# QData/LaMP

Hardware: AMD Instinct MI355X
Metric: forward samples/sec, reuters d512 2+2L 4h (higher is better)
Workload: dtype f32

## Files before the change

### lamp_amd/csrc/chain.hip

```cpp
#include "lamp_asm.h"

namespace lamp {

namespace {
constexpr int ROWS = 16;
constexpr int BK = 32;

}

struct ChainGemm {
    const float* W[3];
    const float* Wp[3];
    const float* Wq[3];
    const float* bias[3];
    float* C[3];
    int nseg, N, K;
    int64_t ldw, ldc;
    int relu;
    int src;
    int dst;
    int add_dst;
};
struct ChainLN {
    const float* g;
// ... 770 lines not shown
    auto buf_f = [&](int which) { return smem + (which ? x_floats : 0); };
    auto buf_w = [&](int which) { return which ? p.hw : d; };

    int pc = 0;
    auto first = [&]() { return (wave - pc) & (WAVES - 1); };
    auto load_rows = [&](const float* src, int64_t ld, int width, int which) {
        const __amdgpu_buffer_rsrc_t rs = rsrc_u(src + row0 * ld, (uint64_t(rows_m - 1) * uint64_t(ld) + uint64_t(width)) * 4u);
        const int ppr = width / 256, n = R * ppr;
        float* dst = buf_f(which);
        const int rl = buf_w(which);
        for (int k = first(); k < n; k += WAVES) {
            const int r = k / ppr, part = k - r * ppr;
            const unsigned voff = unsigned(r) * unsigned(ld) * 4u + unsigned(part * 64 + (lane ^ (r & 15))) * 16u;
            lds_dma16(rs, dst + r * rl + part * 256, r < rows_m ? voff : OOB, 0);
        }
        pc += n;
    };
    auto load_vec = [&](const float* src, int n_floats, int at) {
        const __amdgpu_buffer_rsrc_t rs = rsrc_u(src, uint64_t(n_floats) * 4u);
        const int n = n_floats / 256;
        for (int k = first(); k < n; k += WAVES) lds_dma16(rs, smem + at + k * 256, unsigned(k * 64 + lane) * 16u, 0);
        pc += n;
    };
    auto load_mod_rows = [&](const float* table, int mod, int at, int ld) {
        const __amdgpu_buffer_rsrc_t rs = rsrc_u(table, uint64_t(mod) * uint64_t(d) * 4u);
        const int ppr = d / 256, n = R * ppr;
        for (int k = first(); k < n; k += WAVES) {
            const int r = k / ppr, part = k - r * ppr;
            const unsigned src_row = unsigned(row0 + r) % unsigned(mod);
            lds_dma16(rs, smem + at + r * ld + part * 256, r < rows_m ? (src_row * unsigned(d) + unsigned(part * 64 + lane) * 4u) * 4u : OOB, 0);
        }
        pc += n;
    };
    if (p.in_x) load_rows(p.in_x, d, d, 0);
    load_rows(p.in_h, p.ld_h, p.k_h, 1);
    load_vec(p.ln1.g, d, c_g1);
    load_vec(p.ln1.b, d, c_be1);
    if (p.ln1.res) load_mod_rows(p.ln1.res, p.ln1.r_mod, c_res, res_ld);
    const ChainLN& lnl = p.has_ffn ? p.ln2 : p.ln1;
    if (p.has_ffn) {
        load_vec(p.ln2.g, d, c_g2);
        load_vec(p.ln2.b, d, c_be2);
        load_vec(p.w2.bias[0], d, c_b2);
        load_vec(p.w1.bias[0], dff, c_b1);
    }
    if (lnl.w_out && !p.wout_late) load_mod_rows(lnl.w_out, lnl.n_labels, c_wout, d);
    wait_vmcnt<0>();
    wg_barrier();

#ifdef LAMP_TUNING
    unsigned long long gt[3][4] = {};
    int gt_i = 0;
#endif
    auto gemm = [&](const ChainGemm& g, int bias_at) {
        CHAIN_STAMP(0);
        const int nc = g.K / 16, npass = g.N / 512, total = npass * nc;
        const unsigned w_bytes = unsigned(g.N) * unsigned(g.K) * 4u;
        u32x4 rsW = raw_rsrc(g.Wq[0], w_bytes);
        const unsigned f_voff = unsigned(lane) * 16u;
        const unsigned pass_jump = 7u * unsigned(nc) * 4096u + 4096u;
        unsigned s_off = unsigned(wave) * unsigned(nc) * 4096u;
        int pt = 0, p_kt = 0, p_wrap = 0;
        auto adv_a = [&]() { ++pt; ++p_kt; p_wrap = p_kt == nc ? 1 : 0; };
        auto adv_b = [&]() { s_off += p_wrap ? pass_jump : 4096u; p_kt = p_wrap ? 0 : p_kt; };
        auto adv_c = [&]() {
#if defined(CHAIN_ABL) && (CHAIN_ABL & 1)
            rsW[2] = 0u;
#else
            rsW[2] = pt < total ? w_bytes : 0u;
#endif
        };
        auto wload = [&](f32x4& dst, auto Q) { dst = buffer_read16_untracked_off<decltype(Q)::value * 1024>(rsW, f_voff, s_off); };
        f32x4 F[DEPTH][4];
        float fa[2][G];
        unsigned a_cur[G];
        const unsigned src_b = buf_b(g.src), row_bytes = unsigned(buf_w(g.src)) * 4u;
        const int bq = lane >> 4, be = (lane >> 2) & 3;
        auto a_lane = [&](int gg) { return src_b + unsigned(4 * gg + l3) * row_bytes + unsigned((bq ^ l3) << 4) + unsigned(be) * 4u; };
#pragma unroll
        for (int gg = 0; gg < G; ++gg) a_cur[gg] = a_lane(gg);
        auto aread = [&](auto SET, auto GG, auto J) {
            constexpr int set = decltype(SET)::value, gg = decltype(GG)::value, j = decltype(J)::value;
            fa[set][gg] = lds_read4_off<64 * (j ^ (gg & 3))>(a_cur[gg]);
        };
        static_for<0, DEPTH - 1>([&](auto J) {
            constexpr int j = decltype(J)::value;
            sgpr_guard(rsW, s_off);
            static_for<0, 4>([&](auto Q) { wload(F[j][decltype(Q)::value], Q); });
            adv_a(); adv_b(); adv_c();
        });
        static_for<0, G>([&](auto GG) { aread(std::integral_constant<int, 0>{}, GG, std::integral_constant<int, 0>{}); });
        wait_vmcnt<(DEPTH - 2) * 4>();
        wait_lgkmcnt<0>();
        CHAIN_STAMP(1);
        for (int pass = 0; pass < npass; ++pass) {
            const int col = pass * 512 + wave * 64 + lane;
            f32x4 acc[G];
#pragma unroll
            for (int gg = 0; gg < G; ++gg) acc[gg] = f32x4{0.f, 0.f, 0.f, 0.f};
            for (int kt0 = 0; kt0 < nc; kt0 += DEPTH) {
                const unsigned q_next = unsigned(kt0 + DEPTH == nc ? 0 : (kt0 + DEPTH) >> 2) * 256u;
                static_for<0, DEPTH>([&](auto J) {
                    constexpr int j = decltype(J)::value, set = j & 1, setn = (j + 1) & 1;
                    constexpr int jl = (j + DEPTH - 1) % DEPTH, jn = (j + 1) % DEPTH;
                    static_for<0, NMF>([&](auto I) {
                        constexpr int i = decltype(I)::value, jj = i / (4 * G), q = (i / G) % 4, gg = i % G;
#if !(defined(CHAIN_ABL) && (CHAIN_ABL & 2))
                        acc[gg] = __builtin_amdgcn_mfma_f32_4x4x1f32(fa[set][gg], F[j][q][jj], acc[gg], 4, 4 * q + jj, 0);
#endif
                        __builtin_amdgcn_sched_barrier(0);
                        if constexpr (i < 8 && i % 2 == 0) {
#if !(defined(CHAIN_ABL) && (CHAIN_ABL & 16))
                            wload(F[jl][i / 2], std::integral_constant<int, i / 2>{});
#endif
                        } else if constexpr (i < 2 * G && i % 2 == 1 && i != NMF - 1) {
#if !(defined(CHAIN_ABL) && (CHAIN_ABL & 8))
                            aread(std::integral_constant<int, setn>{}, std::integral_constant<int, i / 2>{}, std::integral_constant<int, jn>{});
#endif
                        } else if constexpr (i == 8) {
                            adv_a();
                        } else if constexpr (i == 10) {
                            adv_b();
                        } else if constexpr (i == 12) {
                            adv_c();
                        } else if constexpr (i >= 14 && i % 2 == 0 && (i - 14) / 2 < G && j == DEPTH - 2) {
                            a_cur[(i - 14) / 2] = a_lane((i - 14) / 2) + q_next;
                        } else if constexpr (i == NMF - 1) {
                            asm volatile("s_waitcnt vmcnt(%0) lgkmcnt(0)" ::"n"((DEPTH - 2) * 4) : "memory");
                        }
                        __builtin_amdgcn_sched_barrier(0);
                    });
                });
            }
            if (pass + 1 == npass) wait_vmcnt<0>();
            static_for<0, DEPTH - 1>([&](auto J) { static_for<0, 4>([&](auto Q) { keep_alive(F[decltype(J)::value][decltype(Q)::value]); }); });
            static_for<0, G>([&](auto GG) { keep_alive(fa[0][decltype(GG)::value]); });
            CHAIN_STAMP(2);
            const unsigned drow = unsigned(buf_w(g.dst)) * 4u;
            float rv[G][4];
            unsigned at[G][4];
#pragma unroll
            for (int gg = 0; gg < G; ++gg)
#pragma unroll
                for (int i = 0; i < 4; ++i) {
                    const int r = 4 * gg + i;
                    at[gg][i] = buf_b(g.dst) + unsigned(r) * drow + unsigned(((col >> 2) ^ (r & 15)) << 4) + unsigned(col & 3) * 4u;
                    rv[gg][i] = lds_read4(at[gg][i]);
                }
            float bias_v = lds_read4(bias_at >= 0 ? lds0 + unsigned(bias_at + col) * 4u : at[0][0]);
            wait_lgkmcnt<0>();
            settle(bias_v);
#pragma unroll
            for (int gg = 0; gg < G; ++gg)
#pragma unroll
                for (int i = 0; i < 4; ++i) settle(rv[gg][i]);
            const float bias = bias_at >= 0 ? bias_v : 0.f;
#pragma unroll
            for (int gg = 0; gg < G; ++gg)
#pragma unroll
                for (int i = 0; i < 4; ++i) {
                    float v = acc[gg][i] + bias;
                    if (g.relu) v = fmaxf(v, 0.f);
                    if (g.add_dst) v = v + rv[gg][i];
                    lds_write4(at[gg][i], v);
                }
        }
        wait_vmcnt<0>();
        wg_barrier();
        CHAIN_STAMP(3);
#ifdef LAMP_TUNING
        ++gt_i;
#endif
    };

    auto layernorm = [&](const ChainLN& n, int g_at, int be_at) {
        const int nv = d / 4;
        int cq[NV];
#pragma unroll
        for (int i = 0; i < NV; ++i) cq[i] = lane + i * 64 < nv ? lane + i * 64 : nv - 1;
#pragma unroll
        for (int q = 0; q < RPW; ++q) {
            const int r = wave + q * WAVES;
            if (r < R) {
                const bool live = r < rows_m;
                const int64_t row = row0 + (live ? r : 0);
                const unsigned row_b = lds0 + unsigned(r) * unsigned(d) * 4u;
                f32x4 raw[NV], gg[NV], bb[NV], rr[NV], ww[NV];
#pragma unroll
                for (int i = 0; i < NV; ++i) {
                    const unsigned self = row_b + unsigned((cq[i] ^ (r & 15)) << 4);
                    raw[i] = lds_read16(self);
                    gg[i] = lds_read16(lds0 + unsigned(g_at) * 4u + unsigned(cq[i]) * 16u);
                    bb[i] = lds_read16(lds0 + unsigned(be_at) * 4u + unsigned(cq[i]) * 16u);
                    rr[i] = lds_read16(n.res ? lds0 + unsigned(c_res + r * res_ld) * 4u + unsigned(cq[i]) * 16u : self);
                    ww[i] = lds_read16(n.w_out ? lds0 + unsigned(c_wout + r * d) * 4u + unsigned(cq[i]) * 16u : self);
                }
                wait_lgkmcnt<0>();
#pragma unroll
                for (int i = 0; i < NV; ++i) {
                    settle(raw[i]); settle(gg[i]); settle(bb[i]); settle(rr[i]); settle(ww[i]);
// ... 5 lines not shown
                    v[i] = in ? make_float4(raw[i].x, raw[i].y, raw[i].z, raw[i].w) : make_float4(0.f, 0.f, 0.f, 0.f);
                    if (n.res && in) {
                        v[i].x += rr[i].x; v[i].y += rr[i].y; v[i].z += rr[i].z; v[i].w += rr[i].w;
                    }
                }
                float mean, rstd;
                ln_row_stats<NV>(v, lane, nv, d, n.eps, mean, rstd);
                float4* yr = (n.y && live) ? reinterpret_cast<float4*>(n.y + row * d) : nullptr;
                float dot = 0.f;
#pragma unroll
                for (int i = 0; i < NV; ++i) {
                    if (lane + i * 64 < nv) {
                        const float4 o = ln_row_apply(v[i], mean, rstd, make_float4(gg[i].x, gg[i].y, gg[i].z, gg[i].w),
                                                      make_float4(bb[i].x, bb[i].y, bb[i].z, bb[i].w));
                        lds_write16(row_b + unsigned((cq[i] ^ (r & 15)) << 4), f32x4{o.x, o.y, o.z, o.w});
                        if (yr) yr[cq[i]] = o;
                        if (n.w_out) dot += dot4_nocontract(o, make_float4(ww[i].x, ww[i].y, ww[i].z, ww[i].w));
                    }
                }
                if (n.w_out) {
                    dot = wave64_sum(dot);
                    if (lane == 0 && live) n.logits[row] = dot;
                }
            }
        }
        wg_barrier();
    };

#ifdef LAMP_TUNING
    unsigned long long t[6] = {};
    const unsigned long long c_begin = __builtin_readcyclecounter();
    if (p.trace) t[0] = wall_clock64();
#endif
    gemm(p.fc, -1);
#ifdef LAMP_TUNING
    if (p.trace) t[1] = wall_clock64();
#endif
    layernorm(p.ln1, c_g1, c_be1);
#ifdef LAMP_TUNING
    if (p.trace) t[2] = wall_clock64();
#endif
    if (p.has_ffn) {
        gemm(p.w1, c_b1);
#ifdef LAMP_TUNING
        if (p.trace) t[3] = wall_clock64();
#endif
        gemm(p.w2, c_b2);
#ifdef LAMP_TUNING
        if (p.trace) t[4] = wall_clock64();
#endif
        if (p.wout_late) {
            load_mod_rows(p.ln2.w_out, p.ln2.n_labels, c_wout, d);
            wait_vmcnt<0>();
            wg_barrier();
        }
        layernorm(p.ln2, c_g2, c_be2);
    }
#ifdef LAMP_TUNING
    if (p.trace && tid == 0) {
        unsigned long long* o = p.trace + size_t(blockIdx.x) * 24;
        t[5] = wall_clock64();
        for (int i = 0; i < 6; ++i) o[i] = t[i];
        o[6] = __builtin_readcyclecounter() - c_begin;
        o[7] = __builtin_amdgcn_s_getreg((31 << 11) | 20);
        for (int gi = 0; gi < 3; ++gi)
            for (int k = 0; k < 4; ++k) o[8 + gi * 4 + k] = gt[gi][k] - c_begin;
    }
#endif
}

#ifdef LAMP_TUNING
static unsigned long long* g_chain_trace = nullptr;
extern "C" __attribute__((visibility("default"))) void lamp_debug_set_chain_trace(unsigned long long* buf) { g_chain_trace = buf; }
static int g_chain_mode = -1;
extern "C" __attribute__((visibility("default"))) void lamp_debug_force_chain(int mode) { g_chain_mode = mode; }
static int g_chain_geom = -1;
extern "C" __attribute__((visibility("default"))) void lamp_debug_chain_geometry(int idx) { g_chain_geom = idx; }
#endif

#define LAMP_CHAIN_GEOMS(X) X(0, 16, 32, 2, 1) X(1, 8, 32, 4, 2) X(2, 8, 32, 2, 2) X(3, 8, 32, 4, 1) X(4, 8, 64, 2, 1) \
// ... 248 lines not shown
```

### lamp_amd/csrc/attention_small.hip

```cpp
#include "lamp_kernels.h"

namespace lamp {

#ifndef LAMP_LDS_PAD16
#define LAMP_LDS_PAD16 8
#endif
constexpr int ATTN16_PAD = LAMP_LDS_PAD16;

namespace {
__device__ __forceinline__ void swap16(float& a, float& b) {
    asm volatile("s_nop 3\n\tv_permlane16_swap_b32 %0, %1\n\ts_nop 3" : "+v"(a), "+v"(b));
}
__device__ __forceinline__ void swap32(float& a, float& b) {
    asm volatile("s_nop 3\n\tv_permlane32_swap_b32 %0, %1\n\ts_nop 3" : "+v"(a), "+v"(b));
}
__device__ __forceinline__ float group_max(float v) {
    float a = v, b = v;
    swap16(a, b);
    a = fmaxf(a, b);
    b = a;
    swap32(a, b);
    return fmaxf(a, b);
}
__device__ __forceinline__ float group_sum(float v) {
    float a = v, b = v;
    swap16(a, b);
    a = a + b;
    b = a;
    swap32(a, b);
    return a + b;
}
}

// ... 277 lines not shown

    if (qi < p.lq) {
        float* Orow = p.O + int64_t(b) * p.lay.o_b + int64_t(h) * p.lay.o_h + int64_t(qi) * p.lay.o_r;
        const bool vec = ((p.lay.o_b | p.lay.o_h | p.lay.o_r) & 3) == 0 && (reinterpret_cast<uintptr_t>(p.O) & 15u) == 0;
#pragma unroll
        for (int r = 0; r < 4; ++r) {
#pragma unroll
            for (int e0 = 0; e0 < DV8; e0 += DVW) {
                const int col = DVW * (4 * g + r) + 64 * (e0 / DVW);
                if (col >= p.dv) continue;
                if (DVW == 4 && vec) {
                    *reinterpret_cast<float4*>(Orow + col) =
                        make_float4(o[e0][r] * inv_l, o[e0 + (DVW > 1 ? 1 : 0)][r] * inv_l,
                                    o[e0 + (DVW > 2 ? 2 : 0)][r] * inv_l, o[e0 + (DVW > 3 ? 3 : 0)][r] * inv_l);
                } else {
#pragma unroll
                    for (int e = 0; e < DVW; ++e) Orow[col + e] = o[e0 + e][r] * inv_l;
                }
            }
        }
    }
#ifdef LAMP_TUNING
    if (p.trace && tid == 0) {
        unsigned long long* t = p.trace + size_t(blockIdx.x) * 8;
        t[0] = t_entry; t[1] = t_loop; t[2] = t_merge; t[3] = wall_clock64();
        t[4] = __builtin_amdgcn_s_getreg((31 << 11) | 4);
        t[5] = __builtin_amdgcn_s_getreg((31 << 11) | 20);
        t[6] = unsigned(item);
        t[7] = unsigned(ks) | (unsigned(qb) << 8);
    }
#endif
}

template <int DP, int QB, int KSPLIT, int PM, int MK>
static int launch_small_mk(const AttnParams& p, hipStream_t s) {
    constexpr int NW = QB * KSPLIT;
    constexpr size_t lds_q = size_t(QB + NW) * 16 * (DP + ATTN16_PAD) * sizeof(float);
    constexpr size_t lds_c = KSPLIT > 1 ? size_t(NW) * (DP / 16 * 4 + 4) * 64 * sizeof(float) : 0;
    constexpr size_t lds = lds_q > lds_c ? lds_q : lds_c;
    auto kern = attn16_kernel<DP, QB, KSPLIT, PM, MK>;
    if constexpr (lds > 65536) {
        static AttrOnce once;
        if (int e = once.set(reinterpret_cast<const void*>(kern), lds)) return e;
    }
    const int64_t nwg = int64_t((p.lq + 16 * QB - 1) / (16 * QB)) * p.H * p.B;
    if (nwg > 0x7fffffffLL) return LAMP_E_DIMS;
    hipLaunchKernelGGL(kern, dim3(unsigned(nwg)), dim3(NW * 64), lds, s, p);
    return int(hipGetLastError());
}

template <int DP, int QB, int KSPLIT, int PM>
static int launch_small_ks(const AttnParams& p, hipStream_t s) {
    switch (p.mask_kind) {
        case LAMP_MASK_U8: return launch_small_mk<DP, QB, KSPLIT, PM, LAMP_MASK_U8>(p, s);
        case LAMP_MASK_KEY_TOKENS_I64: return launch_small_mk<DP, QB, KSPLIT, PM, LAMP_MASK_KEY_TOKENS_I64>(p, s);
        case LAMP_MASK_BITS_U32: return launch_small_mk<DP, QB, KSPLIT, PM, LAMP_MASK_BITS_U32>(p, s);
        default: return launch_small_mk<DP, QB, KSPLIT, PM, LAMP_MASK_NONE>(p, s);
    }
}

template <int DP, int QB, int KSPLIT>
static int launch_small_pm(const AttnParams& p, hipStream_t s) {
    return p.lse ? launch_small_ks<DP, QB, KSPLIT, 2>(p, s) : launch_small_ks<DP, QB, KSPLIT, 0>(p, s);
}

template <int DP>
static int launch_small_dp(const AttnParams& p, int qb, int ksplit, hipStream_t s) {
    switch (qb * 8 + ksplit) {
        case 1 * 8 + 1: return launch_small_pm<DP, 4, 1>(p, s);
        case 2 * 8 + 1: return launch_small_pm<DP, 4, 1>(p, s);
        case 3 * 8 + 1: return launch_small_pm<DP, 4, 1>(p, s);
        case 4 * 8 + 1: return launch_small_pm<DP, 4, 1>(p, s);
        case 1 * 8 + 2: return launch_small_pm<DP, 2, 2>(p, s);
        case 2 * 8 + 2: return launch_small_pm<DP, 2, 2>(p, s);
        case 3 * 8 + 2: return launch_small_pm<DP, 3, 2>(p, s);
        case 4 * 8 + 2: return launch_small_pm<DP, 4, 2>(p, s);
        case 1 * 8 + 4: return launch_small_pm<DP, 1, 4>(p, s);
        case 2 * 8 + 4: return launch_small_pm<DP, 2, 4>(p, s);
        case 3 * 8 + 4: return launch_small_pm<DP, 3, 4>(p, s);
        default: return launch_small_pm<DP, 2, 4>(p, s);
    }
}

bool attn_small_applies(const AttnParams& p, bool any_lq) {
    const bool few_keys = p.lk <= 64 && !p.kv_len;
    return (p.lq <= 256 || few_keys || any_lq) && p.V && p.O && (!p.P || p.lse) && p.dk <= 128 && p.dv <= 128;
}

#ifdef LAMP_TUNING
static unsigned long long* g_attn_trace = nullptr;
extern "C" __attribute__((visibility("default"))) void lamp_debug_set_attn_trace(unsigned long long* buf) { g_attn_trace = buf; }
#endif

int launch_attn_small(const AttnParams& p_in, int force, hipStream_t s) {
    AttnParams p = p_in;
    p.trace = nullptr;
#ifdef LAMP_TUNING
    p.trace = g_attn_trace;
#endif
    const int nt = (p.lk + 15) / 16;
    const int nqb = (p.lq + 15) / 16;
    int ksplit = force & 7;
    if (ksplit != 1 && ksplit != 2 && ksplit != 4) ksplit = nt >= 12 ? 4 : (nt >= 4 ? 2 : 1);
    int qb = (force >> 4) & 7;
    if (qb < 1 || qb > 4) qb = 4 / ksplit;
    (void)nqb;
    const int dmax = p.dk > p.dv ? p.dk : p.dv;
    if (dmax <= 32) return launch_small_dp<32>(p, qb, ksplit, s);
    if (dmax <= 64) return launch_small_dp<64>(p, qb, ksplit, s);
    return launch_small_dp<128>(p, qb, ksplit, s);
}

}
```

### lamp_amd/csrc/attention_tile.hip

```cpp
#include "lamp_asm.h"

namespace lamp {
namespace {

constexpr int TILE_FLOATS = 32 * 128;
constexpr int BUF_FLOATS = 2 * TILE_FLOATS;
constexpr int MAX_LIST_TILES = 2048;
constexpr size_t LDS_BYTES = size_t(2) * BUF_FLOATS * 4;
constexpr size_t LDS_BYTES_LIST = LDS_BYTES + (MAX_LIST_TILES / 32) * 4 + MAX_LIST_TILES * 4;

__device__ __forceinline__ void dma16(u32x4 rs, unsigned lds_addr, unsigned voff, unsigned soff) {
    asm volatile("s_mov_b32 m0, %0\n\ts_nop 0\n\tbuffer_load_dwordx4 %1, %2, %3 offen lds" ::"s"(lds_addr), "v"(voff), "s"(rs), "s"(soff)
                 : "memory");
}

template <int MK>
__global__ __launch_bounds__(256, 2) void attn_tile_kernel(AttnParams p) {
    static_assert(MK == LAMP_MASK_NONE || MK == LAMP_MASK_BITS_U32, "the plan's masks");
    constexpr int DKC = 16, DVB = 4;
    extern __shared__ __attribute__((aligned(16))) float smem[];
#ifdef TILE_TRACE
    const unsigned long long t_entry = wall_clock64();
#endif
    const int tid = threadIdx.x, lane = tid & 63, wave = __builtin_amdgcn_readfirstlane(tid >> 6);
    const int l31 = lane & 31, hi = lane >> 5;
    const int nqb = (p.lq + 127) / 128;
    const int item = xcd_remap(blockIdx.x, gridDim.x);
    const int qblk = item % nqb, bh = item / nqb;
    const int h = bh % p.H, b = bh / p.H;
    const int q0 = (qblk * 4 + wave) * 32;
    const int qi = q0 + l31;
    const bool wave_active = q0 < p.lq;
    const int qc = qi < p.lq ? qi : p.lq - 1;

    const int q_r = int(p.lay.q_r), k_r = int(p.lay.k_r), v_r = int(p.lay.v_r);
    const int lk_b = __builtin_amdgcn_readfirstlane(p.kv_len ? p.kv_len[b] : p.lk);
    const int row0 = __builtin_amdgcn_readfirstlane(p.kv_len ? p.kv_off[b] : 0);
    const int64_t k_row0 = p.kv_len ? int64_t(row0) * k_r : int64_t(b) * p.lay.k_b;
    const int64_t v_row0 = p.kv_len ? int64_t(row0) * v_r : int64_t(b) * p.lay.v_b;
    const __amdgpu_buffer_rsrc_t rsQ = make_rsrc(p.Q + int64_t(b) * p.lay.q_b + int64_t(h) * p.lay.q_h,
                                                 (uint64_t(p.lq - 1) * q_r + p.dk) * 4u);
    const u32x4 rsK = raw_rsrc(p.K + k_row0 + int64_t(h) * p.lay.k_h, lk_b > 0 ? unsigned((uint64_t(lk_b - 1) * k_r + p.dk) * 4u) : 0u);
    const u32x4 rsV = raw_rsrc(p.V + v_row0 + int64_t(h) * p.lay.v_h, lk_b > 0 ? unsigned((uint64_t(lk_b - 1) * v_r + p.dv) * 4u) : 0u);
    const u32x4 rsM = MK == LAMP_MASK_BITS_U32
                          ? raw_rsrc(reinterpret_cast<const float*>(static_cast<const unsigned*>(p.mask) + int64_t(b) * p.m_sb),
                                     unsigned((uint64_t(p.lq - 1) * uint64_t(p.m_sq) + (p.lk + 31) / 32) * 4u))
                          : raw_rsrc(p.K, 0u);
// ... 330 lines not shown
```

### lamp_amd/csrc/lamp_asm.h

```cpp
#pragma once
#include <type_traits>

#include "lamp_kernels.h"

namespace lamp {
namespace {
typedef __attribute__((address_space(3))) void* lds_ptr;
__device__ __forceinline__ void lds_dma16(__amdgpu_buffer_rsrc_t rs, float* dst, unsigned voff, unsigned soff) {
    __builtin_amdgcn_raw_ptr_buffer_load_lds(rs, (lds_ptr)dst, 16, voff, soff, 0, 0);
}
__device__ __forceinline__ f32x4 lds_read16(unsigned addr) {
    f32x4 v;
    asm volatile("ds_read_b128 %0, %1" : "=v"(v) : "v"(addr));
    return v;
}
__device__ __forceinline__ f32x4 global_read16_untracked(const float* ptr) {
    f32x4 v;
    asm volatile("global_load_dwordx4 %0, %1, off" : "=v"(v) : "v"(ptr) : "memory");
    return v;
}
typedef unsigned u32x4 __attribute__((ext_vector_type(4)));
__device__ __forceinline__ u32x4 raw_rsrc(const float* base, unsigned bytes) {
    const uint64_t b = reinterpret_cast<uint64_t>(base);
    return u32x4{unsigned(__builtin_amdgcn_readfirstlane(unsigned(b))), unsigned(__builtin_amdgcn_readfirstlane(unsigned(b >> 32) & 0xffffu)),
                 unsigned(__builtin_amdgcn_readfirstlane(bytes)), 0x00020000u};
}
__device__ __forceinline__ f32x4 buffer_read16_untracked(u32x4 rs, unsigned voff, unsigned soff) {
    f32x4 v;
    asm volatile("buffer_load_dwordx4 %0, %1, %2, %3 offen" : "=v"(v) : "v"(voff), "s"(rs), "s"(soff) : "memory");
    return v;
}
__device__ __forceinline__ void lds_write16(unsigned addr, f32x4 v) { asm volatile("ds_write_b128 %0, %1" ::"v"(addr), "v"(v) : "memory"); }
template <int I, int N, typename F>
__device__ __forceinline__ void static_for(F&& f) {
    if constexpr (I < N) {
        f(std::integral_constant<int, I>{});
        static_for<I + 1, N>(f);
    }
}
template <int N>
__device__ __forceinline__ void wait_vmcnt() { asm volatile("s_waitcnt vmcnt(%0)" ::"n"(N) : "memory"); }
template <int N>
__device__ __forceinline__ void wait_lgkmcnt() {
    asm volatile("s_waitcnt lgkmcnt(%0)" ::"n"(N) : "memory");
    __builtin_amdgcn_sched_barrier(0);
}
__device__ __forceinline__ void wg_barrier() {
    asm volatile("s_waitcnt lgkmcnt(0)" ::: "memory");
    __builtin_amdgcn_s_barrier();
    asm volatile("" ::: "memory");
    __builtin_amdgcn_sched_barrier(0);
}
__device__ __forceinline__ const float* uniform_ptr(const float* q) {
    const uint64_t b = reinterpret_cast<uint64_t>(q);
    const unsigned lo = __builtin_amdgcn_readfirstlane(unsigned(b)), hi = __builtin_amdgcn_readfirstlane(unsigned(b >> 32));
    return reinterpret_cast<const float*>((uint64_t(hi) << 32) | lo);
}
__device__ __forceinline__ __amdgpu_buffer_rsrc_t rsrc_u(const float* base, uint64_t bytes) {
// ... 48 lines not shown
```

### lamp_amd/isa_guard.py

```python
import os
import re
import subprocess
import sys
import tempfile

HIPCC = os.environ.get('HIPCC') or '/opt/rocm/bin/hipcc'

LOAD = re.compile(r'^\s*(buffer_load_dword\w*|global_load_dword\w*|ds_read\w*)\s+(v\[\d+:\d+\]|v\d+)\s*,\s*(.*)$')
REG = re.compile(r'v\[(\d+):(\d+)\]|v(\d+)')


def regs_of(text):
    out = set()
    for m in REG.finditer(text):
        if m.group(3) is not None:
            out.add(int(m.group(3)))
        else:
            out.update(range(int(m.group(1)), int(m.group(2)) + 1))
    return out


def device_asm(path, extra=()):
    if path.endswith('.s'):
        return open(path).read()
# ... 120 lines not shown
            continue
        ops = t.split(None, 1)
        if len(ops) < 2 or ops[0].startswith('s_'):
            continue
        operands = ops[1].split(';')[0]
        parts = [p.strip() for p in operands.split(',')]
        is_store = ops[0].startswith(('ds_write', 'buffer_store', 'global_store', 'scratch_store', 'buffer_load'))
        srcs = pk_sources(parts) if ops[0].startswith('v_pk_') else regs_of(','.join(parts if is_store else parts[1:]))
        dsts = set() if is_store else regs_of(parts[0])
        for regs, lno, ltxt in all_pending():
            if regs & srcs:
                findings.append((kernel, lno, ltxt, no, t))
            elif regs & dsts:
                findings.append((kernel, lno, ltxt, no, t + '   ; WRITES a register in flight'))
    return kernels, n_loads, findings


def m0_findings(asm):
    lines = [l.strip() for l in asm.split('\n')]
    uses = [i for i, l in enumerate(lines) if re.search(r'\bm0\b', l) and not l.startswith(';')]
    bad = []
    for i in uses:
        ok = (lines[i].startswith('s_mov_b32 m0, s') and i + 2 < len(lines) and lines[i + 1].startswith('s_nop') and
              lines[i + 2].startswith('buffer_load_dwordx4') and lines[i + 2].endswith('lds'))
        if not ok:
            bad.append((i + 1, lines[i]))
    n_dma = sum(l.endswith(' lds') and l.startswith('buffer_load') for l in lines)
    if n_dma != len(uses):
        bad.append((0, '%d LDS-DMA loads for %d m0 writes' % (n_dma, len(uses))))
    return len(uses), bad


GUARDED = {'chain.hip': (('chain',), 12, 500, False), 'slab.hip': (('slab',), 1, 500, False),
           'attention_tile.hip': (('attn_tile',), 2, 3, True)}


def guard_unit(path, flags=()):
    unit = os.path.basename(path)
    wanted, min_kernels, min_loads, owns_m0 = GUARDED[unit]
    asm = device_asm(path, flags)
    kernels, loads, findings = check(asm, wanted)
    out = ['%s: line %d `%s` <- line %d `%s`' % (k[:80], lno, ltxt, no, t) for k, lno, ltxt, no, t in findings]
    if kernels < min_kernels or loads <= min_loads:
        out.append('%s: only %d kernels / %d inline-assembly loads seen: the checker no longer recognises the unit' % (unit, kernels, loads))
    if owns_m0:
        n, bad = m0_findings(asm)
        out += ['%s: m0 at line %d: %s' % (unit, no, t) for no, t in bad]
        if n <= 20:
            out.append('%s: only %d m0 writes seen' % (unit, n))
    return out


def main():
    path = sys.argv[1] if len(sys.argv) > 1 else 'lamp_amd/csrc/chain.hip'
    wanted = tuple(sys.argv[2:]) or ('chain', 'slab')
    kernels, n_loads, findings = check(device_asm(path), wanted)
    print('%d kernels, %d inline-assembly loads checked, %d findings' % (kernels, n_loads, len(findings)))
    for k, lno, ltxt, no, t in findings[:40]:
        print('  %s\n    line %d: %s\n    line %d: %s' % (k[:90], lno, ltxt, no, t))
    sys.exit(1 if findings else 0)


if __name__ == '__main__':
    main()
```

Before: 46950.

## Prefetch next GEMM's weight tiles across chain stages and hoist first prefetch

Moves the weight register pipeline F out of the gemm lambda so its prologue prefetch for the first GEMM is issued before the activation/LN-parameter loads. At the tail of each GEMM the buffer descriptor switches to the next GEMM's weights, so the first DEPTH-1 tiles of the following GEMM stream in during the epilogue and layernorm rather than after a full drain. This hides cold-start weight latency between chained stages. The cost is more complex descriptor logic and in-flight loads held across barriers and layernorm, which raises register pressure and adds a correctness risk around the vmcnt waits.

```diff
diff --git a/lamp_amd/csrc/chain.hip b/lamp_amd/csrc/chain.hip
--- a/lamp_amd/csrc/chain.hip
+++ b/lamp_amd/csrc/chain.hip
@@ -826,6 +826,21 @@
         }
         pc += n;
     };
+    f32x4 F[DEPTH][4];
+    auto w_rsrc = [&](const ChainGemm& g, bool live) { return raw_rsrc(g.Wq[0], live ? unsigned(g.N) * unsigned(g.K) * 4u : 0u); };
+    auto w_first = [&](const ChainGemm& g) { return unsigned(wave) * unsigned(g.K / 16) * 4096u; };
+    {
+        const u32x4 rs = w_rsrc(p.fc, true);
+        const unsigned s0 = w_first(p.fc);
+        static_for<0, DEPTH - 1>([&](auto J) {
+            constexpr int j = decltype(J)::value;
+            const unsigned so = s0 + unsigned(j) * 4096u;
+            sgpr_guard(rs, so);
+            static_for<0, 4>([&](auto Q) {
+                F[j][decltype(Q)::value] = buffer_read16_untracked_off<decltype(Q)::value * 1024>(rs, unsigned(lane) * 16u, so);
+            });
+        });
+    }
     if (p.in_x) load_rows(p.in_x, d, d, 0);
     load_rows(p.in_h, p.ld_h, p.k_h, 1);
     load_vec(p.ln1.g, d, c_g1);
@@ -846,26 +861,30 @@
     unsigned long long gt[3][4] = {};
     int gt_i = 0;
 #endif
-    auto gemm = [&](const ChainGemm& g, int bias_at) {
+    auto gemm = [&](const ChainGemm& g, int bias_at, const ChainGemm& nx, bool has_next) {
         CHAIN_STAMP(0);
         const int nc = g.K / 16, npass = g.N / 512, total = npass * nc;
         const unsigned w_bytes = unsigned(g.N) * unsigned(g.K) * 4u;
-        u32x4 rsW = raw_rsrc(g.Wq[0], w_bytes);
+        u32x4 rsW = w_rsrc(g, true);
+        const u32x4 rsN = w_rsrc(nx, has_next);
+        const unsigned n_first = w_first(nx);
         const unsigned f_voff = unsigned(lane) * 16u;
         const unsigned pass_jump = 7u * unsigned(nc) * 4096u + 4096u;
-        unsigned s_off = unsigned(wave) * unsigned(nc) * 4096u;
-        int pt = 0, p_kt = 0, p_wrap = 0;
+        unsigned s_off = w_first(g) + unsigned(DEPTH - 1) * 4096u;
+        int pt = DEPTH - 1, p_kt = DEPTH - 1, p_wrap = 0;
         auto adv_a = [&]() { ++pt; ++p_kt; p_wrap = p_kt == nc ? 1 : 0; };
-        auto adv_b = [&]() { s_off += p_wrap ? pass_jump : 4096u; p_kt = p_wrap ? 0 : p_kt; };
+        auto adv_b = [&]() { s_off = pt == total ? n_first : s_off + (p_wrap ? pass_jump : 4096u); p_kt = p_wrap ? 0 : p_kt; };
         auto adv_c = [&]() {
+            const bool past = pt >= total;
+            rsW[0] = past ? rsN[0] : rsW[0];
+            rsW[1] = past ? rsN[1] : rsW[1];
 #if defined(CHAIN_ABL) && (CHAIN_ABL & 1)
             rsW[2] = 0u;
 #else
-            rsW[2] = pt < total ? w_bytes : 0u;
+            rsW[2] = past ? rsN[2] : w_bytes;
 #endif
         };
         auto wload = [&](f32x4& dst, auto Q) { dst = buffer_read16_untracked_off<decltype(Q)::value * 1024>(rsW, f_voff, s_off); };
-        f32x4 F[DEPTH][4];
         float fa[2][G];
         unsigned a_cur[G];
         const unsigned src_b = buf_b(g.src), row_bytes = unsigned(buf_w(g.src)) * 4u;
@@ -877,12 +896,6 @@
             constexpr int set = decltype(SET)::value, gg = decltype(GG)::value, j = decltype(J)::value;
             fa[set][gg] = lds_read4_off<64 * (j ^ (gg & 3))>(a_cur[gg]);
         };
-        static_for<0, DEPTH - 1>([&](auto J) {
-            constexpr int j = decltype(J)::value;
-            sgpr_guard(rsW, s_off);
-            static_for<0, 4>([&](auto Q) { wload(F[j][decltype(Q)::value], Q); });
-            adv_a(); adv_b(); adv_c();
-        });
         static_for<0, G>([&](auto GG) { aread(std::integral_constant<int, 0>{}, GG, std::integral_constant<int, 0>{}); });
         wait_vmcnt<(DEPTH - 2) * 4>();
         wait_lgkmcnt<0>();
@@ -926,7 +939,7 @@
                     });
                 });
             }
-            if (pass + 1 == npass) wait_vmcnt<0>();
+            if (pass + 1 == npass && !has_next) wait_vmcnt<0>();
             static_for<0, DEPTH - 1>([&](auto J) { static_for<0, 4>([&](auto Q) { keep_alive(F[decltype(J)::value][decltype(Q)::value]); }); });
             static_for<0, G>([&](auto GG) { keep_alive(fa[0][decltype(GG)::value]); });
             CHAIN_STAMP(2);
@@ -959,7 +972,6 @@
                     lds_write4(at[gg][i], v);
                 }
         }
-        wait_vmcnt<0>();
         wg_barrier();
         CHAIN_STAMP(3);
 #ifdef LAMP_TUNING
@@ -1031,7 +1043,7 @@
     const unsigned long long c_begin = __builtin_readcyclecounter();
     if (p.trace) t[0] = wall_clock64();
 #endif
-    gemm(p.fc, -1);
+    gemm(p.fc, -1, p.w1, p.has_ffn != 0);
 #ifdef LAMP_TUNING
     if (p.trace) t[1] = wall_clock64();
 #endif
@@ -1040,11 +1052,11 @@
     if (p.trace) t[2] = wall_clock64();
 #endif
     if (p.has_ffn) {
-        gemm(p.w1, c_b1);
+        gemm(p.w1, c_b1, p.w2, true);
 #ifdef LAMP_TUNING
         if (p.trace) t[3] = wall_clock64();
 #endif
-        gemm(p.w2, c_b2);
+        gemm(p.w2, c_b2, p.w2, false);
 #ifdef LAMP_TUNING
         if (p.trace) t[4] = wall_clock64();
 #endif
```

After: 47150, median of 6. Within noise of the previous version (+0.4%).

## Add LDS-staged small attention kernel sharing K/V tiles across query blocks via DMA

Applied to the files above, without the earlier changes.

Adds a new small-attention kernel in which each key-split wave group loads K/V tiles into LDS through buffer-load-to-LDS DMA and a double/triple-buffered ring. Three query blocks then read the same tile, so K/V global traffic is no longer repeated per query block. This becomes the default path when there is no LSE output and the key split is greater than one. In exchange it adds more LDS use per workgroup, barriers on every step in the non-burst case, and a fixed QB=3 choice; the ISA guard is extended to cover the new m0 usage.

```diff
diff --git a/lamp_amd/csrc/attention_small.hip b/lamp_amd/csrc/attention_small.hip
--- a/lamp_amd/csrc/attention_small.hip
+++ b/lamp_amd/csrc/attention_small.hip
@@ -1,4 +1,4 @@
-#include "lamp_kernels.h"
+#include "lamp_asm.h"
 
 namespace lamp {
 
@@ -342,6 +342,308 @@
 #endif
 }
 
+template <int DP, int QB, int KSPLIT, int NBUF, int MK>
+__global__ __launch_bounds__(QB* KSPLIT * 64) void attn16_lds_kernel(AttnParams p) {
+    static_assert(KSPLIT > 1 && NBUF >= 2, "shared tiles need a key split; the ring needs two buffers");
+    constexpr int DKC = DP / 16, DV8 = DP / 16;
+    constexpr int QS = DP + ATTN16_PAD;
+    constexpr int C4 = DP / 4, RPI = 64 / C4;
+    constexpr int SWM = (C4 < 16 ? C4 : 16) - 1;
+    constexpr int TILE = 16 * DP;
+    constexpr int NREQ = TILE * 4 / 1024;
+    constexpr int QFL = QB * 16 * QS;
+    extern __shared__ __attribute__((aligned(16))) float smem[];
+
+    const int tid = threadIdx.x;
+    const int lane = tid & 63, wave = __builtin_amdgcn_readfirstlane(tid >> 6);
+    const int l15 = lane & 15, g = lane >> 4;
+    const int rot = (p.kv_len) ? int(blockIdx.x % KSPLIT) : 0;
+    const int qb = wave / KSPLIT, ks = __builtin_amdgcn_readfirstlane((wave % KSPLIT + KSPLIT - rot) % KSPLIT);
+    const int slot = qb * KSPLIT + ks;
+#ifdef LAMP_TUNING
+    const unsigned long long t_entry = p.trace ? wall_clock64() : 0ull;
+    unsigned long long t_loop = 0, t_merge = 0;
+#endif
+    const int nqg = (p.lq + 16 * QB - 1) / (16 * QB);
+    const int item = xcd_remap(blockIdx.x, gridDim.x);
+    const int qgrp = item % nqg;
+    const int bh = item / nqg;
+    const int h = bh % p.H, b = bh / p.H;
+    const int q0 = (qgrp * QB + qb) * 16;
+    const int qi = q0 + l15;
+    const bool wave_active = q0 < p.lq;
+    const int qc = qi < p.lq ? qi : p.lq - 1;
+
+    const int q_r = int(p.lay.q_r), k_r = int(p.lay.k_r), v_r = int(p.lay.v_r);
+    const int lk_b = __builtin_amdgcn_readfirstlane(p.kv_len ? p.kv_len[b] : p.lk);
+    const int row0 = __builtin_amdgcn_readfirstlane(p.kv_len ? p.kv_off[b] : 0);
+    const int64_t k_row0 = p.kv_len ? int64_t(row0) * k_r : int64_t(b) * p.lay.k_b;
+    const int64_t v_row0 = p.kv_len ? int64_t(row0) * v_r : int64_t(b) * p.lay.v_b;
+    const __amdgpu_buffer_rsrc_t rsQ = make_rsrc(p.Q + int64_t(b) * p.lay.q_b + int64_t(h) * p.lay.q_h,
+                                                 (uint64_t(p.lq - 1) * q_r + p.dk) * 4u);
+    const u32x4 rsK = raw_rsrc(p.K + k_row0 + int64_t(h) * p.lay.k_h, lk_b > 0 ? unsigned((uint64_t(lk_b - 1) * k_r + p.dk) * 4u) : 0u);
+    const u32x4 rsV = raw_rsrc(p.V + v_row0 + int64_t(h) * p.lay.v_h, lk_b > 0 ? unsigned((uint64_t(lk_b - 1) * v_r + p.dv) * 4u) : 0u);
+    const __amdgpu_buffer_rsrc_t rsM =
+        MK == LAMP_MASK_BITS_U32
+            ? make_rsrc(static_cast<const unsigned*>(p.mask) + int64_t(b) * p.m_sb,
+                        (uint64_t(p.lq - 1) * uint64_t(p.m_sq) + (p.lk + 31) / 32) * 4u)
+        : MK == LAMP_MASK_U8
+            ? make_rsrc(static_cast<const unsigned char*>(p.mask) + int64_t(b) * p.m_sb,
+                        uint64_t(p.lq - 1) * uint64_t(p.m_sq) + p.lk)
+        : MK == LAMP_MASK_KEY_TOKENS_I64
+            ? make_rsrc(static_cast<const long long*>(p.mask) + int64_t(b) * p.m_sb, uint64_t(p.lk) * 8u)
+            : make_rsrc(p.K, 0);
+
+    const int nt_b = (lk_b + 15) / 16;
+    const int nt = nt_b;
+    const int ks_eff = p.kv_len ? (nt_b >= 12 ? (KSPLIT < 4 ? KSPLIT : 4) : (nt_b >= 4 ? 2 : 1)) : KSPLIT;
+    const int nsteps = nt > 0 ? (nt + ks_eff - 1) / ks_eff : 0;
+    const bool burst = nsteps <= NBUF;
+
+    unsigned kvo[NREQ];
+#pragma unroll
+    for (int i = 0; i < NREQ; ++i) {
+        const int r = i * RPI + lane / C4, q = (lane % C4) ^ (r & SWM);
+        kvo[i] = 4 * q < p.dk ? unsigned((lane / C4) * k_r + 4 * q) * 4u : OOB;
+    }
+    const unsigned vvo = 4 * (lane % C4) < p.dv ? unsigned((lane / C4) * v_r + 4 * (lane % C4)) * 4u : OOB;
+    auto buf_of = [&](int u) { return QFL + (ks * NBUF + u) * 2 * TILE; };
+    auto dma_tile = [&](int j, int u) {
+        const int kt = ks + j * ks_eff;
+        if (ks >= ks_eff || kt >= nt) return;
+        const unsigned base = unsigned(buf_of(u)) * 4u;
+#pragma unroll
+        for (int n = 0; n < 2 * NREQ; ++n) {
+            if (n % QB != qb) continue;
+            if (n < NREQ) dma16(rsK, base + 1024u * n, kvo[n], unsigned((kt * 16 + n * RPI) * k_r) * 4u);
+            else dma16(rsV, base + TILE * 4u + 1024u * (n - NREQ), vvo, unsigned((kt * 16 + (n - NREQ) * RPI) * v_r) * 4u);
+        }
+    };
+    sgpr_guard(rsK);
+    sgpr_guard(rsV);
+    if (burst) {
+        for (int j = 0; j < nsteps; ++j) dma_tile(j, j);
+    } else {
+        dma_tile(0, 0);
+    }
+
+    float* Qs = smem + qb * 16 * QS;
+    {
+        constexpr int PER_WAVE = 16 * C4 / KSPLIT;
+#pragma unroll
+        for (int i = 0; i < (PER_WAVE + 63) / 64; ++i) {
+            const int idx = ks * PER_WAVE + i * 64 + lane;
+            const int row = idx / C4, c = (idx - row * C4) * 4;
+            const int q = q0 + row;
+            if (i * 64 + lane < PER_WAVE) {
+                const float4 v = bload4(rsQ, (q < p.lq && c < p.dk) ? unsigned(q * q_r + c) * 4u : OOB, 0);
+                *reinterpret_cast<float4*>(Qs + row * QS + c) =
+                    make_float4(v.x * p.scale_log2e, v.y * p.scale_log2e, v.z * p.scale_log2e, v.w * p.scale_log2e);
+            }
+        }
+    }
+
+    unsigned mbits = 0;
+    const unsigned m_voff = unsigned(int64_t(qc) * p.m_sq) * 4u;
+    auto load_mask = [&](int kt) {
+        const int kbase = kt * 16 + 4 * g;
+        if constexpr (MK == LAMP_MASK_BITS_U32) {
+            mbits = __builtin_amdgcn_raw_buffer_load_b32(rsM, m_voff, unsigned(kt >> 1) * 4u, 0);
+        } else if constexpr (MK == LAMP_MASK_U8) {
+            const unsigned mo = unsigned(int64_t(qc) * p.m_sq) + unsigned(kbase);
+            unsigned m = 0;
+#pragma unroll
+            for (int r = 0; r < 4; ++r) m |= (bload_u8(rsM, kt < nt ? mo + r : OOB) != 0 ? 1u : 0u) << r;
+            mbits = m;
+        } else if constexpr (MK == LAMP_MASK_KEY_TOKENS_I64) {
+            unsigned m = 0;
+#pragma unroll
+            for (int r = 0; r < 4; ++r) m |= (bload_u64(rsM, unsigned(kbase + r) * 8u) == 0 ? 1u : 0u) << r;
+            mbits = m;
+        }
+    };
+    const bool work = wave_active && ks < ks_eff && ks < nt;
+    if (work) load_mask(ks);
+    wait_vmcnt<0>();
+    __syncthreads();
+
+    int koff[DKC];
+#pragma unroll
+    for (int c = 0; c < DKC; ++c) koff[c] = l15 * DP + 4 * ((4 * c + g) ^ (l15 & SWM));
+    constexpr int DVW = DV8 == 8 ? 4 : DV8;
+    const int voff = 4 * g * DP + DVW * l15;
+
+    f32x4 o[DV8];
+#pragma unroll
+    for (int e = 0; e < DV8; ++e) o[e] = f32x4{0.f, 0.f, 0.f, 0.f};
+    float m_run = -INFINITY, l_part = 0.f;
+    constexpr float RESCALE_THR = 32.0f;
+
+#ifdef LAMP_TUNING
+    if (p.trace) t_loop = wall_clock64();
+#endif
+    for (int j = 0; j < nsteps; ++j) {
+        const int kt = ks + j * ks_eff;
+        const bool mine = work && kt < nt;
+        const float* Kt = smem + buf_of(burst ? j : (j & 1));
+        const float* Vt = Kt + TILE;
+        f32x4 s0, s1 = {0.f, 0.f, 0.f, 0.f};
+        if (mine) {
+            const int valid = lk_b - kt * 16;
+            const unsigned tail = valid >= 16 ? 0u : (0xffffu << (valid > 0 ? valid : 0)) & 0xffffu;
+            unsigned word = tail;
+            if constexpr (MK == LAMP_MASK_BITS_U32) word |= mbits >> ((kt & 1) * 16);
+            const int mine_bits = MK == LAMP_MASK_BITS_U32 || MK == LAMP_MASK_NONE ? int(word >> (4 * g)) : int(mbits | (tail >> (4 * g)));
+#pragma unroll
+            for (int r = 0; r < 4; ++r) {
+                int t;
+                asm("v_bfe_i32 %0, %1, %2, 1" : "=v"(t) : "v"(mine_bits), "n"(r));
+                s0[r] = __int_as_float(t & int(0xff800000u));
+            }
+        }
+        __builtin_amdgcn_sched_barrier(0);
+        if (!burst && j + 1 < nsteps) dma_tile(j + 1, (j + 1) & 1);
+        __builtin_amdgcn_sched_barrier(0);
+        if (mine) {
+            const float* qp = Qs + l15 * QS + 4 * g;
+#pragma unroll
+            for (int c = 0; c < DKC; c += 2) {
+                const float4 qa = *reinterpret_cast<const float4*>(qp + 16 * c);
+                const float4 qb2 = *reinterpret_cast<const float4*>(qp + 16 * c + 16);
+                const float4 ka = *reinterpret_cast<const float4*>(Kt + koff[c]);
+                const float4 kb = *reinterpret_cast<const float4*>(Kt + koff[c + 1]);
+                s0 = __builtin_amdgcn_mfma_f32_16x16x4f32(ka.x, qa.x, s0, 0, 0, 0);
+                s1 = __builtin_amdgcn_mfma_f32_16x16x4f32(kb.x, qb2.x, s1, 0, 0, 0);
+                s0 = __builtin_amdgcn_mfma_f32_16x16x4f32(ka.y, qa.y, s0, 0, 0, 0);
+                s1 = __builtin_amdgcn_mfma_f32_16x16x4f32(kb.y, qb2.y, s1, 0, 0, 0);
+                s0 = __builtin_amdgcn_mfma_f32_16x16x4f32(ka.z, qa.z, s0, 0, 0, 0);
+                s1 = __builtin_amdgcn_mfma_f32_16x16x4f32(kb.z, qb2.z, s1, 0, 0, 0);
+                s0 = __builtin_amdgcn_mfma_f32_16x16x4f32(ka.w, qa.w, s0, 0, 0, 0);
+                s1 = __builtin_amdgcn_mfma_f32_16x16x4f32(kb.w, qb2.w, s1, 0, 0, 0);
+            }
+            f32x4 s;
+#pragma unroll
+            for (int r = 0; r < 4; ++r) s[r] = s0[r] + s1[r];
+            load_mask(kt + ks_eff);
+            const float tmax = fmaxf(fmaxf(s[0], s[1]), fmaxf(s[2], s[3]));
+            if (__any(tmax > m_run + RESCALE_THR)) {
+                const float m_new = fmaxf(m_run, group_max(tmax));
+                const float alpha = __builtin_amdgcn_exp2f(m_run - ((m_new == -INFINITY) ? 0.f : m_new));
+                l_part *= alpha;
+                m_run = m_new;
+#pragma unroll
+                for (int e = 0; e < DV8; ++e)
+#pragma unroll
+                    for (int r = 0; r < 4; ++r) o[e][r] *= alpha;
+            }
+            const float m_use = (m_run == -INFINITY) ? 0.f : m_run;
+#pragma unroll
+            for (int r = 0; r < 4; ++r) s[r] = __builtin_amdgcn_exp2f(s[r] - m_use);
+            l_part += (s[0] + s[1]) + (s[2] + s[3]);
+#pragma unroll
+            for (int r = 0; r < 4; ++r) {
+                float vf[DV8];
+                const float* vp = Vt + voff + r * DP;
+                if constexpr (DV8 == 8) {
+                    const float4 a = *reinterpret_cast<const float4*>(vp);
+                    const float4 c2 = *reinterpret_cast<const float4*>(vp + 64);
+                    vf[0] = a.x; vf[1] = a.y; vf[2] = a.z; vf[3] = a.w;
+                    vf[4] = c2.x; vf[5] = c2.y; vf[6] = c2.z; vf[7] = c2.w;
+                } else if constexpr (DV8 == 4) {
+                    const float4 a = *reinterpret_cast<const float4*>(vp);
+                    vf[0] = a.x; vf[1] = a.y; vf[2] = a.z; vf[3] = a.w;
+                } else {
+                    const f32x2 a = *reinterpret_cast<const f32x2*>(vp);
+                    vf[0] = a.x; vf[1] = a.y;
+                }
+#pragma unroll
+                for (int e = 0; e < DV8; ++e) o[e] = __builtin_amdgcn_mfma_f32_16x16x4f32(vf[e], s[r], o[e], 0, 0, 0);
+            }
+        }
+        if (!burst) {
+            wait_vmcnt<0>();
+            __syncthreads();
+        }
+    }
+
+#ifdef LAMP_TUNING
+    if (p.trace) t_merge = wall_clock64();
+#endif
+    {
+        constexpr int CW = (DV8 * 4 + 4) * 64;
+        __syncthreads();
+        float* mine = smem + slot * CW;
+#pragma unroll
+        for (int e = 0; e < DV8; ++e)
+            *reinterpret_cast<float4*>(mine + (e * 64 + lane) * 4) = make_float4(o[e][0], o[e][1], o[e][2], o[e][3]);
+        *reinterpret_cast<float4*>(mine + (DV8 * 64 + lane) * 4) = make_float4(m_run, l_part, 0.f, 0.f);
+        __syncthreads();
+        if (ks == 0 && wave_active) {
+            float m_all = m_run;
+#pragma unroll
+            for (int s2 = 1; s2 < KSPLIT; ++s2)
+                if (s2 < ks_eff) m_all = fmaxf(m_all, smem[(slot + s2) * CW + (DV8 * 64 + lane) * 4]);
+            const float m_use = (m_all == -INFINITY) ? 0.f : m_all;
+            const float w0 = exp2f(m_run - m_use);
+            l_part *= w0;
+#pragma unroll
+            for (int e = 0; e < DV8; ++e)
+#pragma unroll
+                for (int r = 0; r < 4; ++r) o[e][r] *= w0;
+#pragma unroll
+            for (int s2 = 1; s2 < KSPLIT; ++s2) {
+                if (s2 >= ks_eff) break;
+                const float* other = smem + (slot + s2) * CW;
+                const float4 ml = *reinterpret_cast<const float4*>(other + (DV8 * 64 + lane) * 4);
+                const float ws = exp2f(ml.x - m_use);
+                l_part = fmaf(ml.y, ws, l_part);
+#pragma unroll
+                for (int e = 0; e < DV8; ++e) {
+                    const float4 v = *reinterpret_cast<const float4*>(other + (e * 64 + lane) * 4);
+                    o[e][0] = fmaf(v.x, ws, o[e][0]);
+                    o[e][1] = fmaf(v.y, ws, o[e][1]);
+                    o[e][2] = fmaf(v.z, ws, o[e][2]);
+                    o[e][3] = fmaf(v.w, ws, o[e][3]);
+                }
+            }
+            m_run = m_all;
+        }
+    }
+    if (!(wave_active && ks == 0)) return;
+    const float l_run = group_sum(l_part);
+    const float inv_l = 1.0f / l_run;
+    if (qi < p.lq) {
+        float* Orow = p.O + int64_t(b) * p.lay.o_b + int64_t(h) * p.lay.o_h + int64_t(qi) * p.lay.o_r;
+        const bool vec = ((p.lay.o_b | p.lay.o_h | p.lay.o_r) & 3) == 0 && (reinterpret_cast<uintptr_t>(p.O) & 15u) == 0;
+#pragma unroll
+        for (int r = 0; r < 4; ++r) {
+#pragma unroll
+            for (int e0 = 0; e0 < DV8; e0 += DVW) {
+                const int col = DVW * (4 * g + r) + 64 * (e0 / DVW);
+                if (col >= p.dv) continue;
+                if (DVW == 4 && vec) {
+                    *reinterpret_cast<float4*>(Orow + col) =
+                        make_float4(o[e0][r] * inv_l, o[e0 + (DVW > 1 ? 1 : 0)][r] * inv_l,
+                                    o[e0 + (DVW > 2 ? 2 : 0)][r] * inv_l, o[e0 + (DVW > 3 ? 3 : 0)][r] * inv_l);
+                } else {
+#pragma unroll
+                    for (int e = 0; e < DVW; ++e) Orow[col + e] = o[e0 + e][r] * inv_l;
+                }
+            }
+        }
+    }
+#ifdef LAMP_TUNING
+    if (p.trace && tid == 0) {
+        unsigned long long* t = p.trace + size_t(blockIdx.x) * 8;
+        t[0] = t_entry; t[1] = t_loop; t[2] = t_merge; t[3] = wall_clock64();
+        t[4] = __builtin_amdgcn_s_getreg((31 << 11) | 4);
+        t[5] = __builtin_amdgcn_s_getreg((31 << 11) | 20);
+        t[6] = unsigned(item);
+        t[7] = unsigned(ks) | (unsigned(qb) << 8);
+    }
+#endif
+}
+
 template <int DP, int QB, int KSPLIT, int PM, int MK>
 static int launch_small_mk(const AttnParams& p, hipStream_t s) {
     constexpr int NW = QB * KSPLIT;
@@ -367,6 +669,39 @@
         case LAMP_MASK_BITS_U32: return launch_small_mk<DP, QB, KSPLIT, PM, LAMP_MASK_BITS_U32>(p, s);
         default: return launch_small_mk<DP, QB, KSPLIT, PM, LAMP_MASK_NONE>(p, s);
     }
+}
+
+template <int DP, int QB, int KSPLIT, int NBUF, int MK>
+static int launch_lds_mk(const AttnParams& p, hipStream_t s) {
+    constexpr int NW = QB * KSPLIT;
+    constexpr size_t lds_t = (size_t(QB) * 16 * (DP + ATTN16_PAD) + size_t(KSPLIT) * NBUF * 2 * 16 * DP) * sizeof(float);
+    constexpr size_t lds_c = size_t(NW) * (DP / 16 * 4 + 4) * 64 * sizeof(float);
+    constexpr size_t lds = lds_t > lds_c ? lds_t : lds_c;
+    static_assert(lds <= 160 * 1024, "one workgroup per CU");
+    auto kern = attn16_lds_kernel<DP, QB, KSPLIT, NBUF, MK>;
+    if constexpr (lds > 65536) {
+        static AttrOnce once;
+        if (int e = once.set(reinterpret_cast<const void*>(kern), lds)) return e;
+    }
+    const int64_t nwg = int64_t((p.lq + 16 * QB - 1) / (16 * QB)) * p.H * p.B;
+    if (nwg > 0x7fffffffLL) return LAMP_E_DIMS;
+    hipLaunchKernelGGL(kern, dim3(unsigned(nwg)), dim3(NW * 64), lds, s, p);
+    return int(hipGetLastError());
+}
+
+template <int DP, int KSPLIT, int NBUF>
+static int launch_lds_ks(const AttnParams& p, hipStream_t s) {
+    switch (p.mask_kind) {
+        case LAMP_MASK_U8: return launch_lds_mk<DP, 3, KSPLIT, NBUF, LAMP_MASK_U8>(p, s);
+        case LAMP_MASK_KEY_TOKENS_I64: return launch_lds_mk<DP, 3, KSPLIT, NBUF, LAMP_MASK_KEY_TOKENS_I64>(p, s);
+        case LAMP_MASK_BITS_U32: return launch_lds_mk<DP, 3, KSPLIT, NBUF, LAMP_MASK_BITS_U32>(p, s);
+        default: return launch_lds_mk<DP, 3, KSPLIT, NBUF, LAMP_MASK_NONE>(p, s);
+    }
+}
+
+template <int DP>
+static int launch_lds_dp(const AttnParams& p, int ksplit, hipStream_t s) {
+    return ksplit == 4 ? launch_lds_ks<DP, 4, 2>(p, s) : launch_lds_ks<DP, 2, 3>(p, s);
 }
 
 template <int DP, int QB, int KSPLIT>
@@ -416,6 +751,11 @@
     if (qb < 1 || qb > 4) qb = 4 / ksplit;
     (void)nqb;
     const int dmax = p.dk > p.dv ? p.dk : p.dv;
+    if (!p.lse && ksplit > 1 && !(force & 0x400) && ((force >> 4) & 7) == 0) {
+        if (dmax <= 32) return launch_lds_dp<32>(p, ksplit, s);
+        if (dmax <= 64) return launch_lds_dp<64>(p, ksplit, s);
+        return launch_lds_dp<128>(p, ksplit, s);
+    }
     if (dmax <= 32) return launch_small_dp<32>(p, qb, ksplit, s);
     if (dmax <= 64) return launch_small_dp<64>(p, qb, ksplit, s);
     return launch_small_dp<128>(p, qb, ksplit, s);
diff --git a/lamp_amd/csrc/attention_tile.hip b/lamp_amd/csrc/attention_tile.hip
--- a/lamp_amd/csrc/attention_tile.hip
+++ b/lamp_amd/csrc/attention_tile.hip
@@ -8,11 +8,6 @@
 constexpr int MAX_LIST_TILES = 2048;
 constexpr size_t LDS_BYTES = size_t(2) * BUF_FLOATS * 4;
 constexpr size_t LDS_BYTES_LIST = LDS_BYTES + (MAX_LIST_TILES / 32) * 4 + MAX_LIST_TILES * 4;
-
-__device__ __forceinline__ void dma16(u32x4 rs, unsigned lds_addr, unsigned voff, unsigned soff) {
-    asm volatile("s_mov_b32 m0, %0\n\ts_nop 0\n\tbuffer_load_dwordx4 %1, %2, %3 offen lds" ::"s"(lds_addr), "v"(voff), "s"(rs), "s"(soff)
-                 : "memory");
-}
 
 template <int MK>
 __global__ __launch_bounds__(256, 2) void attn_tile_kernel(AttnParams p) {
diff --git a/lamp_amd/csrc/lamp_asm.h b/lamp_amd/csrc/lamp_asm.h
--- a/lamp_amd/csrc/lamp_asm.h
+++ b/lamp_amd/csrc/lamp_asm.h
@@ -24,6 +24,10 @@
     const uint64_t b = reinterpret_cast<uint64_t>(base);
     return u32x4{unsigned(__builtin_amdgcn_readfirstlane(unsigned(b))), unsigned(__builtin_amdgcn_readfirstlane(unsigned(b >> 32) & 0xffffu)),
                  unsigned(__builtin_amdgcn_readfirstlane(bytes)), 0x00020000u};
+}
+__device__ __forceinline__ void dma16(u32x4 rs, unsigned lds_addr, unsigned voff, unsigned soff) {
+    asm volatile("s_mov_b32 m0, %0\n\ts_nop 0\n\tbuffer_load_dwordx4 %1, %2, %3 offen lds" ::"s"(lds_addr), "v"(voff), "s"(rs), "s"(soff)
+                 : "memory");
 }
 __device__ __forceinline__ f32x4 buffer_read16_untracked(u32x4 rs, unsigned voff, unsigned soff) {
     f32x4 v;
diff --git a/lamp_amd/isa_guard.py b/lamp_amd/isa_guard.py
--- a/lamp_amd/isa_guard.py
+++ b/lamp_amd/isa_guard.py
@@ -176,7 +176,7 @@
 
 
 GUARDED = {'chain.hip': (('chain',), 12, 500, False), 'slab.hip': (('slab',), 1, 500, False),
-           'attention_tile.hip': (('attn_tile',), 2, 3, True)}
+           'attention_tile.hip': (('attn_tile',), 2, 3, True), 'attention_small.hip': (('attn16_lds',), 24, -1, True)}
 
 
 def guard_unit(path, flags=()):
```

Result: slower. 46600 before, 45750 after (median of 2 runs) (-1.8%).
